# TheShinning/gps-sdr-sim

Hardware: AMD Instinct MI355X
Metric: IQ MSamples/s (and × real-time) at 2.6 MS/s, 12 sats, -b 16; 1/2/4/8 GPU (higher is better)
Workload: dtype int64 phases + f16 x f16 -> f32 MFMA accumulate (exact integer sums)

## Files before the change

### gps-sdr-sim_amd/csrc/common/gss_lin.h

```cpp
#ifndef GSS_LIN_H
#define GSS_LIN_H

#include <stdint.h>

#ifndef GSS_LIN_CH
#define GSS_LIN_CH     16
#endif
#define GSS_LIN_CHUNK  (64 * GSS_LIN_CH)
#define GSS_LIN_SEG    4096

#if defined(__HIPCC__)
#define GSS_LIN_FN static __host__ __device__ inline
#else
#define GSS_LIN_FN static inline
#endif

#define GSS_LIN_CSH    26

GSS_LIN_FN uint32_t gss_lin_dx(uint64_t xs) { return (uint32_t)((xs * 64u + (1ull << 31)) >> 32); }
GSS_LIN_FN uint32_t gss_lin_dz(uint64_t zs)
{
    return (uint32_t)((zs * 64u + (1ull << (GSS_LIN_CSH - 1))) >> GSS_LIN_CSH);
}
GSS_LIN_FN uint64_t gss_lin_xa(uint64_t xs)
// ... 4 lines not shown
GSS_LIN_FN uint64_t gss_lin_za(uint64_t zs)
{
    const int64_t ec = (int64_t)(((uint64_t)gss_lin_dz(zs) << GSS_LIN_CSH) - zs * 64u);
    return (1ull << (GSS_LIN_CSH - 1)) - (uint64_t)((ec * (GSS_LIN_CH - 1)) / 2);
}

GSS_LIN_FN uint32_t gss_lin_e0(uint64_t chips)
{
    const uint32_t e = (uint32_t)(chips % 1023u);
    return e ? e : 1023u;
}

#define GSS_LIN_KDEV_CARR(zs)                                                                      \
    ((((uint64_t)GSS_LIN_CH / 2 + 3) << 31) +                                                     \
     ((2 + (((uint64_t)gss_lin_dz(zs) * (GSS_LIN_CH - 1)) >> 32)) << 32))
#define GSS_LIN_KDEV_CODE (((uint64_t)GSS_LIN_CH / 2 + 3) << (GSS_LIN_CSH - 1))
#define GSS_LIN_WIN_OK(zs) ((zs) * 63u + (3ull << 50) <= (31ull << 50))

#define GSS_LIN_TWE     2560
#define GSS_LIN_CBW_PRE 2
GSS_LIN_FN uint32_t gss_lin_wstep16(int n_per_blk)
{
    return (uint32_t)((104755200ull + (uint64_t)n_per_blk / 2) / (uint64_t)n_per_blk);
}
GSS_LIN_FN int gss_lin_win16_ok(uint64_t zs, int n_per_blk)
{
    const int64_t U = (int64_t)1 << 50, z = (int64_t)zs;
    const int64_t kd = (int64_t)GSS_LIN_KDEV_CODE + ((int64_t)1 << 27);
    const uint32_t w = gss_lin_wstep16(n_per_blk);
    if (zs == 0 || zs >= (uint64_t)U)
        return 0;
    for (int s = 0; s < GSS_LIN_CH; s++) {
        const int64_t f = (int64_t)(((uint64_t)s * w) >> 4) - GSS_LIN_CBW_PRE;
        if (64 * s * z - kd < f * U)
            return 0;
        if (U + (64 * s + 63) * z + kd > (f + 32) * U)
            return 0;
    }
    return 1025 * U + (int64_t)(GSS_LIN_SEG - GSS_LIN_CHUNK) * z + kd < (int64_t)GSS_LIN_TWE * U;
}

GSS_LIN_FN uint64_t gss_lin_lane(uint64_t xs, uint64_t zs, uint32_t l)
{
    const uint32_t lx = (uint32_t)(((uint64_t)l * xs + (1ull << 31)) >> 32);
    const uint32_t lz = (uint32_t)(((uint64_t)l * zs) >> GSS_LIN_CSH);
    return ((uint64_t)lx << 32) | lz;
// ... 147 lines not shown
```

### gps-sdr-sim_amd/csrc/hip/gss_dev.h

```cpp
#ifndef GSS_DEV_H
#define GSS_DEV_H

#include <hip/hip_runtime.h>
#include <stdint.h>
#include "gpssim_amd.h"
#include "../common/gss_impair.h"

extern "C" int gss_fail(int code, const char *fmt, ...);

#define HIP_TRY(x)                                                                           \
    do {                                                                                     \
        hipError_t e_ = (x);                                                                 \
        if (e_ != hipSuccess)                                                                \
            return gss_fail(GSS_E_HIP, "HIP error %s at %s:%d", hipGetErrorString(e_),      \
                            __FILE__, __LINE__);                                             \
    } while (0)

template <class T> struct gss_buf {
    T *p = nullptr;
    size_t cap = 0;
    int reserve(size_t bytes, const char *what)
    {
        if (bytes <= cap)
            return 0;
        release();
        if (hipMalloc((void **)&p, bytes) != hipSuccess) {
            p = nullptr;
            return gss_fail(GSS_E_NOMEM, "%s: %zu bytes of device memory", what, bytes);
        }
// ... 15 lines not shown
    uint32_t ca[32 * GSS_CA_WORDS];
    int16_t lut[1024];
    int32_t noise[GSS_IMP_TBL];
};

struct gss_trk_state;

struct gss_dev {
    int ordinal;
    int seg_r = 1024;
    struct anchor_set {
        gss_buf<double> carr, code;
        gss_buf<uint32_t> cnt;
    } set[2];
    static constexpr int RING = 256;
    hipEvent_t ev_a[RING][2], ev_b[RING][2];
    hipEvent_t ev_l[RING][2];
    int n_a = 0, n_b = 0, n_l = 0;
    lut_arg lut;
    gss_buf<gss_dev_tables> tab;
    gss_buf<uint8_t> d_in, d_out;
    gss_buf<double> d_cend;
    gss_buf<uint32_t> d_cbw;
    gss_buf<int32_t> d_status;
    hipStream_t aux = nullptr;
    hipEvent_t ev_in = nullptr, ev_fb = nullptr;
    struct {
        gss_buf<int8_t> planes, rep;
        gss_buf<uint64_t> rows, cand;
        gss_buf<int32_t> maxes;
    } acq;
    struct {
        gss_buf<gss_trk_state> state;
        gss_buf<gss_trk_job_t> jobs;
    } trk;
};

#endif
```

### gps-sdr-sim_amd/csrc/hip/gss_run.hip

```cpp
#include <hip/hip_runtime.h>
#include <math.h>
#include <stdint.h>
#include <stdlib.h>
#include <stdio.h>
#include <string.h>
#include <time.h>
#include <condition_variable>
#include <mutex>
#include <thread>
#include <unordered_map>
#include <vector>
#include "gpssim_amd.h"
#include "gss_run_modes.h"

extern "C" int gss_fail(int code, const char *fmt, ...);
extern "C" void gss_pool_select(int id);
extern "C" int gss_jam_check(const gss_jam_t *jam, int n_jam);
int run_copy_launch(void *dst, const void *src, size_t n, hipStream_t st);
extern "C" __attribute__((weak)) int gss_impair_device(gss_dev *d, const gss_impair_t *p,
                                                       const int16_t *iq, uint64_t sample0,
                                                       size_t n, int fmt, void *out,
                                                       void *stream);
extern "C" __attribute__((weak)) int gss_jam_device(gss_dev *d, const gss_impair_t *p,
                                                    const gss_jam_t *jam, int n_jam,
                                                    const int16_t *iq, uint64_t sample0, size_t n,
                                                    int fmt, void *out, void *stream);

#define RUN_TRY(x)                                                                           \
    do {                                                                                     \
        hipError_t e_ = (x);                                                                 \
        if (e_ != hipSuccess)                                                                \
            return gss_fail(GSS_E_HIP, "HIP error %s at %s:%d", hipGetErrorString(e_),      \
                            __FILE__, __LINE__);                                             \
    } while (0)

namespace {

static double tnow()
{
    timespec ts;
    clock_gettime(CLOCK_MONOTONIC, &ts);
    return ts.tv_sec + 1e-9 * ts.tv_nsec;
}
static int trace_on()
{
    static int on = -1;
    if (on < 0) {
        const char *e = getenv("GSS_RUN_TRACE");
        on = e && e[0] == '1';
// ... 239 lines not shown
    hipEvent_t tq = nullptr;
    hipEvent_t tk = nullptr;
    hipEvent_t tc = nullptr;
    hipStream_t pst = nullptr;
    hipEvent_t navd = nullptr;
    hipEvent_t proved = nullptr;
    int gpu_proven = 0;
};

struct Run {
    explicit Run(const RunModes &modes) : m(modes) {}
    const RunModes m;
    gss_scn *scn;
    gss_dev *dev = nullptr;
    int ordinal = 0;
    int batch, threads, n_per_blk, carrier_int;
    int fmt = 0;
    size_t bb = 0, bb_r = 0;
    hipStream_t st = nullptr;
    hipStream_t cp[NCOPY] = {};
    uint32_t *d_ca = nullptr;
    hipStream_t nav_st = nullptr;
    hipEvent_t t_base = nullptr;
    hipEvent_t ca_ready = nullptr;
    int64_t first, last;
    int64_t start = 0;
    const gss_run_opts_t *opts;
    const gss_impair_t *impair = nullptr;
    gss_jam_t jam[GSS_MAXJAM];
    int n_jam = 0;
    int fmt_out = 0;
    std::vector<gss_chan_blk_t> pre_blk;
    std::vector<int32_t> pre_nch;
    std::vector<double> pre_ck;
    int64_t pre_n = 0, pre_at = 0;
    std::mutex mu;
    std::condition_variable cv;
    int abort = 0;
    uint32_t ca[32 * GSS_CA_WORDS];
    int nav_planned = 0;
    uint32_t *d_nav = nullptr;
    size_t d_nav_cap = 0;
    struct SpecBatch {
        std::vector<gss_chan_blk_t> blk;
        std::vector<int32_t> nch;
        std::vector<gss_chain_t> chain;
// ... 1133 lines not shown
    }
}


#define THEN(e, x)                                                                           \
    do {                                                                                     \
        if ((e) == hipSuccess)                                                               \
            (e) = (x);                                                                       \
    } while (0)

int run_alloc(Run &r)
{
    gss_ca_table(r.ca);
    hipError_t e = dev_alloc((void **)&r.d_ca, sizeof r.ca);
    THEN(e, r.m.render_rest ? cu_mask_stream(&r.st, r.m.spec_cus, true) : stream_get(&r.st, false));
    for (hipStream_t &c : r.cp)
        THEN(e, stream_get(&c, false));
    if (trace_on()) {
        THEN(e, hipEventCreate(&r.t_base));
        THEN(e, hipEventRecord(r.t_base, r.st));
    }
    if (e != hipSuccess)
        return gss_fail(GSS_E_HIP, "run setup failed");
    return gss_ca_table_device(r.dev, r.d_ca, r.st);
}

void run_release_tables(Run &r)
{
    dev_free(r.d_ca);
    dev_free(r.d_nav);
}

void run_release_streams(Run &r)
{
    stream_put(r.st);
    for (hipStream_t c : r.cp)
        stream_put(c);
    if (r.t_base) (void)hipEventDestroy(r.t_base);
}

int slot_alloc(const Run &r, Slot &sl)
{
    const size_t nb = (size_t)r.batch;
    const unsigned ev = trace_on() ? hipEventDefault : hipEventDisableTiming;
    hipError_t e = pin_alloc((void **)&sl.blk, sizeof(gss_chan_blk_t) * GSS_MAXCH * nb);
    THEN(e, pin_alloc((void **)&sl.nch, sizeof(int32_t) * nb));
    THEN(e, pin_alloc((void **)&sl.ck, sizeof(double) * GSS_MAXCH * GSS_NCK * nb));
    THEN(e, pool_get((void **)&sl.h_out, r.bb * nb, true, r.ordinal, &sl.h_out_bytes));
    THEN(e, pin_alloc((void **)&sl.h_status, sizeof(int32_t)));
    THEN(e, pool_get((void **)&sl.d_out, r.bb_r * nb, false, r.ordinal, &sl.d_out_bytes));
    if (r.impair && r.fmt != r.fmt_out)
// ... 304 lines not shown
```

### gps-sdr-sim_amd/csrc/hip/gss_synth.hip

```cpp
#include <hip/hip_runtime.h>
#include <stdint.h>
#include <stdlib.h>
#include <string.h>
#include "gpssim_amd.h"
#include "gss_dev.h"
#include "../common/gss_phase.h"
#include "../common/gss_lin.h"

#define SYNTH_THREADS  256
#define SYNTH_WAVES    (SYNTH_THREADS / 64)
#define ANCHOR_THREADS 64
#define CHUNK_BYTES    128
#define CHUNK_PIECES   (CHUNK_BYTES / 16)
#define LUT_N          1024

__global__ __launch_bounds__(ANCHOR_THREADS) void gss_anchor_kernel(
    const gss_chan_blk_t *__restrict__ blk, const int32_t *__restrict__ nch,
    const double *__restrict__ carr_ck, int nblk, int nchp, int n_per_blk, int nseg, int nsegp,
    int seg_r, double *__restrict__ seg_carr, double *__restrict__ seg_code,
    uint32_t *__restrict__ seg_cnt, double *__restrict__ carr_end,
    const int32_t *__restrict__ blist)
{
    const int nsub = carr_ck ? GSS_NCK : 1;
    const int nbw = (nblk + ANCHOR_THREADS - 1) / ANCHOR_THREADS;
// ... 346 lines not shown
                                    (size_t)ch * CHUNK_BYTES + piece * 16;
                    const uint32_t *sp = stg + src * (CHUNK_BYTES / 4) + piece * 4;
                    store16(sdst, make_uint4(sp[0], sp[1], sp[2], sp[3]));
                }
            }
            wave_sync_lds();
        }
        if (!full && nsamp > 0) {
            int nbytes = nsamp * BPS4 / 4;
            uint8_t *bp = dst + (size_t)ch * CHUNK_BYTES;
            const uint8_t *sp = (const uint8_t *)mine;
            for (int i = 0; i < nbytes; i++)
                bp[i] = sp[i];
        }
    }
    if (bad && status)
        atomicOr(status, bad);
}

#define LIN_THREADS 256
#define LIN_WAVES   (LIN_THREADS / 64)
#define LIN_STEPS   (GSS_LIN_SEG / 64)
#define LIN_CH      GSS_LIN_CH
#define CBW_PRE     2
#define CBW_CHIPS   3072
#define CAB_W       ((CBW_CHIPS + 96) / 32)
static_assert(LIN_STEPS % LIN_CH == 0 && (LIN_CH & (LIN_CH - 1)) == 0, "whole chunks");
#define LIN_SW_SGPRS 68
typedef _Float16 lin_half4 __attribute__((ext_vector_type(4)));
typedef _Float16 lin_half8 __attribute__((ext_vector_type(8)));
typedef float lin_f4 __attribute__((ext_vector_type(4)));
#define LIN_GS    2
#define LIN_MAGF  (12582912.0f + 64.0f * LIN_GS)
#define LIN_MAGB  0x4B400000u

#define LIN_CHUNKS (LIN_STEPS / LIN_CH)
struct alignas(16) lin_ck {
    uint64_t B[GSS_MAXCH];
    uint32_t A[GSS_MAXCH / 2][5][4];
};
struct alignas(16) lin_wrec {
    uint64_t D[GSS_MAXCH];
    int32_t gd[GSS_MAXCH];
    int32_t pos1[GSS_MAXCH];
    lin_ck ck[LIN_CHUNKS];
};
static_assert(LIN_CHUNKS * GSS_MAXCH == 64, "one lane per (chunk, channel) record");
static_assert(offsetof(lin_wrec, D) % 16 == 0 && offsetof(lin_wrec, ck) % 16 == 0 &&
              offsetof(lin_ck, B) % 16 == 0 && offsetof(lin_ck, A) % 16 == 0 &&
              sizeof(lin_ck) % 16 == 0, "16-byte reads of a pair's B, D and gain operand");

typedef gss_lin_row lin_seg;
typedef gss_lin_chan lin_chan;
static_assert(sizeof(lin_seg) == 32 && sizeof(lin_chan) == 32, "two 16-byte LDS reads each");

__global__ void gss_cab_kernel(const uint32_t *__restrict__ ca_bits, int n_ca,
                               uint32_t *__restrict__ cab)
{
    const int i = blockIdx.x * blockDim.x + threadIdx.x;
    if (i >= n_ca * CAB_W)
        return;
    const int row = i / CAB_W, j0 = (i - row * CAB_W) * 32 - 32;
    const uint32_t *cb = ca_bits + (size_t)row * GSS_CA_WORDS;
    uint32_t w = 0;
    for (int q = 0; q < 32; q++) {
        const int e = j0 + q, chip = ((e % GSS_CA_LEN) + GSS_CA_LEN) % GSS_CA_LEN;
        w |= (((cb[chip >> 5] >> (chip & 31)) & 1u) ^ 1u) << q;
    }
    cab[i] = w;
}

__global__ void gss_tw16_kernel(const uint32_t *__restrict__ cab, int n_ca, uint32_t w,
                                uint32_t *__restrict__ tw)
{
    const int i = blockIdx.x * blockDim.x + threadIdx.x;
    if (i >= n_ca * GSS_LIN_TWE * LIN_CH)
        return;
    const int row = i / (GSS_LIN_TWE * LIN_CH), r = i - row * (GSS_LIN_TWE * LIN_CH);
    const int E = r / LIN_CH, st = r % LIN_CH;
    const uint32_t j = min((uint32_t)(E + (int)(((uint32_t)st * w) >> 4) - GSS_LIN_CBW_PRE + 32),
                           (uint32_t)(32 * CAB_W - 64));
    const uint32_t *c = cab + (size_t)row * CAB_W;
    const uint32_t lin = __builtin_amdgcn_alignbit(c[(j >> 5) + 1], c[j >> 5], j & 31);
    tw[i] = __builtin_amdgcn_alignbit(lin, lin, (32u - j) & 31u);
}

struct lin_wsrc {
    const uint32_t *W;
};

__device__ __forceinline__ void lin_wissue(const lin_wsrc &w, uint32_t (&ws)[LIN_CH])
{
#pragma unroll
    for (int s = 0; s < LIN_CH; s++)
        ws[s] = w.W[s];
}

__device__ __forceinline__ void lin_wfence(const uint32_t (&ws)[LIN_CH])
{
    static_assert(LIN_CH == 16, "the fence below names 16 windows");
    asm volatile("" :: "s"(ws[0]), "s"(ws[1]), "s"(ws[2]), "s"(ws[3]), "s"(ws[4]), "s"(ws[5]),
                 "s"(ws[6]), "s"(ws[7]), "s"(ws[8]), "s"(ws[9]), "s"(ws[10]), "s"(ws[11]),
                 "s"(ws[12]), "s"(ws[13]), "s"(ws[14]), "s"(ws[15]));
}

__device__ __forceinline__ lin_wsrc lin_wsrc_of(uint32_t wa, const uint32_t *__restrict__ tw)
{
// ... 574 lines not shown
    }
    *out = d;
    return 0;
}

extern "C" int gss_dev_close(gss_dev *d)
{
    if (!d) return 0;
    (void)hipSetDevice(d->ordinal);
    gss_run_pool_drain(d->ordinal);
    for (auto &a : d->set) {
        a.carr.release();
        a.code.release();
        a.cnt.release();
    }
    if (d->aux) (void)hipStreamDestroy(d->aux);
    if (d->ev_in) (void)hipEventDestroy(d->ev_in);
    if (d->ev_fb) (void)hipEventDestroy(d->ev_fb);
    d->tab.release();
    d->d_in.release();
    d->d_out.release();
    d->d_cend.release();
    d->d_cbw.release();
    d->d_status.release();
    d->acq.planes.release();
    d->acq.rep.release();
    d->acq.rows.release();
    d->acq.cand.release();
    d->acq.maxes.release();
    d->trk.state.release();
    d->trk.jobs.release();
    for (int i = 0; i < gss_dev::RING; i++)
        for (int j = 0; j < 2; j++) {
            if (d->ev_a[i][j]) (void)hipEventDestroy(d->ev_a[i][j]);
            if (d->ev_b[i][j]) (void)hipEventDestroy(d->ev_b[i][j]);
            if (d->ev_l[i][j]) (void)hipEventDestroy(d->ev_l[i][j]);
        }
    delete d;
    return 0;
}

static int nseg_of(int n, int r) { return (n + r - 1) / r; }
static int nsegp_of(int n, int r) { return (nseg_of(n, r) + 1 + 31) & ~31; }

static int reserve_set(gss_dev *d, int set, int max_blocks, int n_per_blk, int R)
{
// ... 123 lines not shown
                                 const int32_t *nch, int nch_max, const uint32_t *ca_bits,
                                 int n_ca, const uint32_t *nav, int n_nav, int nblk,
                                 int n_per_blk, int fmt, void *out, int32_t *status, void *stream)
{
    (void)n_ca; (void)n_nav;
    return render_launch(d, set, blk, nch, nch_max, ca_bits, nav, nblk, n_per_blk, fmt, out,
                         status, nullptr, d->seg_r, stream);
}

typedef void (*lin_fn)(const gss_lin_t *, const gss_chan_blk_t *, const int32_t *,
                       const int32_t *, const uint32_t *, const uint32_t *, const uint4 *, int,
                       int, uint8_t *, size_t);

static lin_fn pick_lin(int fmt)
{
    switch (fmt) {
    case 16: return gss_lin_kernel<16>;
    case 8: return gss_lin_kernel<8>;
    case 1: return gss_lin_kernel<1>;
    default: return nullptr;
    }
}

extern "C" int gss_synth_lin_device(gss_dev *d, const gss_chan_blk_t *blk, const int32_t *nch,
                                    int nch_max, const gss_lin_t *lin, const int32_t *fast,
                                    const int32_t *fb_list, int n_fb, const double *carr_ck,
                                    const uint32_t *ca_bits, int n_ca, const uint32_t *nav,
                                    int n_nav, int nblk, int n_per_blk, int fmt, void *out,
                                    int32_t *status, void *stream)
{
    (void)n_nav;
    if (!d || !blk || !nch || !lin || !fast || !ca_bits || !out || nblk <= 0 || n_per_blk <= 0 ||
        n_ca <= 0 || n_fb < 0 || n_fb > nblk || (n_fb > 0 && !fb_list))
        return gss_fail(GSS_E_ARG, "invalid synth_lin arguments");
    const size_t bb = gss_block_bytes(n_per_blk, fmt);
    if (bb == 0)
        return gss_fail(GSS_E_ARG, "invalid format %d for %d samples/block", fmt, n_per_blk);
    const int nchp = nch_max < 1 ? 1 : nch_max;
    if (nchp > GSS_MAXCH)
        return gss_fail(GSS_E_ARG, "nch_max %d > %d", nch_max, GSS_MAXCH);
    lin_fn fn = pick_lin(fmt);
    if (!fn)
        return gss_fail(GSS_E_ARG, "no fast kernel for fmt=%d nch=%d", fmt, nchp);
    HIP_TRY(hipSetDevice(d->ordinal));
    hipStream_t st = (hipStream_t)stream;
    const size_t ncbw = (size_t)n_ca * CAB_W, ntw = (size_t)n_ca * GSS_LIN_TWE * LIN_CH;
    const size_t tw_off = (ncbw + 63) & ~(size_t)63;
    int rc = d->d_cbw.reserve((tw_off + ntw) * sizeof(uint32_t), "chip-sign streams");
    if (rc) return rc;
    hipLaunchKernelGGL(gss_cab_kernel, dim3((unsigned)((ncbw + 255) / 256)), dim3(256), 0, st,
                       ca_bits, n_ca, d->d_cbw.p);
    HIP_TRY(hipGetLastError());
    hipLaunchKernelGGL(gss_tw16_kernel, dim3((unsigned)((ntw + 255) / 256)), dim3(256), 0, st,
                       (const uint32_t *)d->d_cbw.p, n_ca, gss_lin_wstep16(n_per_blk),
                       d->d_cbw.p + tw_off);
    HIP_TRY(hipGetLastError());
    const int segs = (n_per_blk + 64 * LIN_STEPS - 1) / (64 * LIN_STEPS);
    const int wg_per_blk = (segs + LIN_WAVES - 1) / LIN_WAVES;
    if (n_fb > 0) {
        HIP_TRY(hipEventRecord(d->ev_in, st));
        HIP_TRY(hipStreamWaitEvent(d->aux, d->ev_in, 0));
        const int R = 256;
        rc = anchor_launch(d, 0, blk, nch, nch_max, carr_ck, n_fb, n_per_blk, nullptr,
                               fb_list, R, d->aux);
        if (rc) return rc;
        rc = render_launch(d, 0, blk, nch, nch_max, ca_bits, nav, n_fb, n_per_blk, fmt, out,
                           status, fb_list, R, d->aux);
        if (rc) return rc;
        HIP_TRY(hipEventRecord(d->ev_fb, d->aux));
    }
    hipEvent_t *ev = d->ev_l[d->n_l % gss_dev::RING];
    d->n_l++;
    HIP_TRY(hipEventRecord(ev[0], st));
    hipLaunchKernelGGL(fn, dim3((unsigned)nblk * wg_per_blk), dim3(LIN_THREADS), 0, st, lin,
                       blk, nch, fast, d->d_cbw.p, d->d_cbw.p + tw_off, (const uint4 *)d->tab.p->lut16,
                       n_per_blk, wg_per_blk, (uint8_t *)out, bb);
    HIP_TRY(hipGetLastError());
    HIP_TRY(hipEventRecord(ev[1], st));
    if (n_fb > 0)
        HIP_TRY(hipStreamWaitEvent(st, d->ev_fb, 0));
    return 0;
}

extern "C" int gss_synth_device(gss_dev *d, const gss_chan_blk_t *blk, const int32_t *nch,
                                int nch_max, const double *carr_ck, const uint32_t *ca_bits,
                                int n_ca,
                                const uint32_t *nav, int n_nav, int nblk, int n_per_blk, int fmt,
                                void *out, double *carr_end, int32_t *status, void *stream)
{
    if (!d || !blk || !nch || !ca_bits || !out || nblk <= 0 || n_per_blk <= 0)
        return gss_fail(GSS_E_ARG, "invalid synth arguments");
    if (gss_block_bytes(n_per_blk, fmt) == 0)
        return gss_fail(GSS_E_ARG, "invalid format %d for %d samples/block", fmt, n_per_blk);
    int rc = gss_anchor_device(d, 0, blk, nch, nch_max, carr_ck, nblk, n_per_blk, carr_end,
                               stream);
    if (rc) return rc;
    return gss_render_device(d, 0, blk, nch, nch_max, ca_bits, n_ca, nav, n_nav, nblk, n_per_blk,
                             fmt, out, status, stream);
// ... 166 lines not shown
```

### gps-sdr-sim_amd/gpssim_amd/__init__.py

```python
import ctypes as C
import os

import numpy as np

PKG_DIR = os.path.dirname(os.path.dirname(os.path.abspath(__file__)))
REPO_DIR = os.path.dirname(PKG_DIR)
_INTREE = os.path.join(PKG_DIR, "lib", "libgpssim_amd.so")
if os.environ.get("GSS_LIB_PATH") and os.environ.get("GSS_ALLOW_LIB_OVERRIDE") != "1":
    raise ImportError("GSS_LIB_PATH is set without GSS_ALLOW_LIB_OVERRIDE=1: refusing to load a "
                      "library other than the in-tree build " + _INTREE)
LIB_PATH = os.environ.get("GSS_LIB_PATH") or _INTREE
IN_TREE = os.path.abspath(LIB_PATH) == os.path.abspath(_INTREE)
CLI_PATH = os.path.join(PKG_DIR, "bin", "gps-sdr-sim")
ACQ_CLI_PATH = os.path.join(PKG_DIR, "bin", "gps-sdr-acq")
TRK_CLI_PATH = os.path.join(PKG_DIR, "bin", "gps-sdr-track")
PVT_CLI_PATH = os.path.join(PKG_DIR, "bin", "gps-sdr-pvt")

MAXCH = 16
CA_WORDS = 32
NAV_WORDS = 60
NCK = 8
FMT_SC01, FMT_SC08, FMT_SC16 = 1, 8, 16

CHAN_DTYPE = np.dtype([
# ... 196 lines not shown
SINK_FN = C.CFUNCTYPE(C.c_int, C.c_void_p, C.c_void_p, C.c_size_t, C.c_int64, C.c_int)
_SIGS = {
    "gss_run": (C.c_int, [_P, _P, C.c_int64, C.c_int64, C.c_int, C.c_int, SINK_FN, _P]),
    "gss_run_ex": (C.c_int, [_P, _P, C.c_int64, C.c_int64, C.c_int, C.c_int, SINK_FN, _P, _P]),
    "gss_dev_open": (C.c_int, [C.POINTER(_P), C.c_int]),
    "gss_dev_close": (C.c_int, [_P]),
    "gss_dev_reserve": (C.c_int, [_P, C.c_int, C.c_int]),
    "gss_block_bytes": (C.c_size_t, [C.c_int, C.c_int]),
    "gss_anchor_device": (C.c_int, [_P, C.c_int, _P, _P, C.c_int, _P, C.c_int, C.c_int, _P,
                                    _P]),
    "gss_render_device": (C.c_int, [_P, C.c_int, _P, _P, C.c_int, _P, C.c_int, _P, C.c_int,
                                    C.c_int, C.c_int, C.c_int, _P, _P, _P]),
    "gss_synth_device": (C.c_int, [_P, _P, _P, C.c_int, _P, _P, C.c_int, _P, C.c_int,
                                   C.c_int, C.c_int, C.c_int, _P, _P, _P, _P]),
    "gss_synth_host": (C.c_int, [_P, _P, _P, _P, _P, C.c_int, _P, C.c_int, C.c_int, C.c_int,
                                 C.c_int, _P, _P]),
    "gss_linearize": (C.c_int, [_P, _P, C.c_int, C.c_int, _P, C.c_int, _P, C.c_int, _P, _P,
                                C.c_int]),
    "gss_linearize_device": (C.c_int, [_P, _P, _P, C.c_int, C.c_int, _P, C.c_int, _P, C.c_int, _P,
                                       _P, _P]),
    "gss_synth_lin_device": (C.c_int, [_P, _P, _P, C.c_int, _P, _P, _P, C.c_int, _P, _P,
                                       C.c_int, _P, C.c_int, C.c_int, C.c_int, C.c_int, _P, _P,
                                       _P]),
    "gss_minmax_mod": (None, [C.c_uint64, C.c_uint64, C.c_uint64, C.c_uint64,
                              C.POINTER(C.c_uint64), C.POINTER(C.c_uint64)]),
    "gss_first_below": (C.c_uint64, [C.c_uint64] * 5),
    "gss_hits_mod": (C.c_int, [C.c_uint64] * 5 + [_P, C.c_int, C.c_int]),
    "gss_noise_table": (C.c_int, [_P]),
    "gss_impair_host": (C.c_int, [C.POINTER(Impair), _P, C.c_uint64, C.c_size_t, C.c_int, _P]),
    "gss_impair_device": (C.c_int, [_P, C.POINTER(Impair), _P, C.c_uint64, C.c_size_t, C.c_int,
                                    _P, _P]),
    "gss_jam_make": (C.c_int, [C.c_double] * 7 + [C.POINTER(Jam)]),
    "gss_jam_host": (C.c_int, [C.POINTER(Impair), C.POINTER(Jam), C.c_int, _P, C.c_uint64,
                               C.c_size_t, C.c_int, _P]),
    "gss_jam_device": (C.c_int, [_P, C.POINTER(Impair), C.POINTER(Jam), C.c_int, _P, C.c_uint64,
                                 C.c_size_t, C.c_int, _P, _P]),
    "gss_acq_sizes": (C.c_int, [C.POINTER(Acq), C.POINTER(C.c_int32), C.POINTER(C.c_int32),
                                C.POINTER(C.c_int64), C.POINTER(C.c_int32),
                                C.POINTER(C.c_int32)]),
    "gss_acquire_host": (C.c_int, [C.POINTER(Acq), _P, _P, _P, C.POINTER(C.c_int), C.c_int]),
    "gss_acquire_device": (C.c_int, [_P, C.POINTER(Acq), _P, _P, _P, _P, _P]),
    "gss_acquire": (C.c_int, [_P, C.POINTER(Acq), _P, _P, _P, C.POINTER(C.c_int)]),
    "gss_acq_expect": (C.c_int, [_P, C.c_double, C.c_int64, C.POINTER(_Truth)]),
    "gss_acq_threshold": (C.c_double, [C.c_int, C.c_uint64, C.c_double]),
    "gss_trk_defaults": (C.c_int, [C.c_int32, C.c_int32, C.POINTER(Trk)]),
    "gss_trk_job_from_peak": (C.c_int, [C.POINTER(Acq), _P, C.c_int64, C.c_int32, _P]),
# ... 686 lines not shown
        return (out, cend) if want_carr_end else out

    def synth_device(self, blk_ptr, nch_ptr, nch_max, ca_ptr, n_ca, nav_ptr, n_nav, nblk,
                     n_per_blk, fmt, out_ptr, carr_end_ptr=0, status_ptr=0, stream=0, ck_ptr=0):
        _check(lib().gss_synth_device(self._h, blk_ptr, nch_ptr, nch_max, ck_ptr or None, ca_ptr,
                                      n_ca, nav_ptr,
                                      n_nav, nblk, n_per_blk, fmt, out_ptr,
                                      carr_end_ptr or None, status_ptr or None, stream or None))

    def ca_table_device(self, out_ptr, stream=0):
        _check(lib().gss_ca_table_device(self._h, out_ptr, stream or None))

    def nav_rows_device(self, src_ptr, first, n, rows_ptr, stream=0):
        _check(lib().gss_nav_rows_device(self._h, src_ptr, first, n, rows_ptr, stream or None))

    def synth_lin_device(self, blk_ptr, nch_ptr, nch_max, lin_ptr, fast_ptr, fb_ptr, n_fb, ca_ptr,
                         n_ca, nav_ptr, n_nav, nblk, n_per_blk, fmt, out_ptr, status_ptr=0,
                         stream=0, ck_ptr=0):
        _check(lib().gss_synth_lin_device(self._h, blk_ptr, nch_ptr, nch_max, lin_ptr, fast_ptr,
                                          fb_ptr or None, n_fb, ck_ptr or None, ca_ptr, n_ca,
                                          nav_ptr, n_nav, nblk, n_per_blk, fmt, out_ptr,
                                          status_ptr or None, stream or None))

    def timing_lin(self):
        n, t = C.c_int(), C.c_float()
        _check(lib().gss_dev_timing_lin(self._h, C.byref(n), C.byref(t)))
        return n.value, t.value

    def anchor_device(self, set_, blk_ptr, nch_ptr, nch_max, nblk, n_per_blk, ck_ptr=0,
                      carr_end_ptr=0, stream=0):
        _check(lib().gss_anchor_device(self._h, set_, blk_ptr, nch_ptr, nch_max, ck_ptr or None,
                                       nblk, n_per_blk, carr_end_ptr or None, stream or None))

    def render_device(self, set_, blk_ptr, nch_ptr, nch_max, ca_ptr, n_ca, nav_ptr, n_nav, nblk,
                      n_per_blk, fmt, out_ptr, status_ptr=0, stream=0):
        _check(lib().gss_render_device(self._h, set_, blk_ptr, nch_ptr, nch_max, ca_ptr, n_ca,
                                       nav_ptr, n_nav, nblk, n_per_blk, fmt, out_ptr,
                                       status_ptr or None, stream or None))

    def impair_device(self, imp, iq_ptr, sample0, n, fmt, out_ptr, stream=0):
        _check(lib().gss_impair_device(self._h, C.byref(imp), C.c_void_p(iq_ptr), int(sample0),
                                       int(n), int(fmt), C.c_void_p(out_ptr),
                                       C.c_void_p(stream or None)))

    def jam_device(self, imp, jam, iq_ptr, sample0, n, fmt, out_ptr, stream=0):
        arr, nj = _jam_array(jam)
# ... 116 lines not shown
```

### gps-sdr-sim_amd/gpssim_amd/render.py

```python
import time

import numpy as np

from . import (CHAN_DTYPE, LIN_DTYPE, MAXCH, NCK, block_bytes, ca_table, carr_advance_ck,
               linearize)


def block_checkpoints(blk, nch, n_per_blk, blocks=None):
    ck = np.zeros((len(nch), MAXCH, NCK), np.float64)
    for b in (range(len(nch)) if blocks is None else blocks):
        for k in range(int(nch[b])):
            ck[b, k] = carr_advance_ck(float(blk[b, k]["carr0"]), float(blk[b, k]["carr_step"]),
                                       n_per_blk)[1]
    return ck


class DeviceWindow:

    def __init__(self, torch, dev, dev_t, blk, nch, nav, n_per_blk, fmt, ck=None, threads=8,
                 batch=3000, out=None, proof="gpu", sizes=None):
        self.torch, self.dev, self.fmt, self.npb = torch, dev, fmt, n_per_blk

        def up(a):
            return torch.from_numpy(np.ascontiguousarray(a).view(np.uint8).reshape(-1)).to(dev_t)

        t0 = time.perf_counter()
        if proof == "gpu":
            self.d_blk, self.d_nch = up(blk), up(np.asarray(nch, np.int32))
            ca = ca_table()
            self.d_ca, self.d_nav = up(ca), up(nav)
            nb = len(nch)
            self.d_lin = torch.empty(max(1, nb * MAXCH * LIN_DTYPE.itemsize), dtype=torch.uint8,
                                     device=dev_t)
            d_fast = torch.empty(max(1, nb), dtype=torch.int32, device=dev_t)
            stream = torch.cuda.current_stream(dev_t).cuda_stream
            if nb:
                dev.linearize_device(self.d_blk.data_ptr(), self.d_nch.data_ptr(), nb, n_per_blk,
                                     self.d_ca.data_ptr(), len(ca), self.d_nav.data_ptr(),
                                     len(nav), self.d_lin.data_ptr(), d_fast.data_ptr(), stream)
            fast = d_fast[:nb].cpu().numpy()
            lin = None
        else:
            lin, fast = linearize(blk, nch, nav, n_per_blk, threads=threads)
        self.lin_s = time.perf_counter() - t0
        self.proof = proof
        self.nblk = len(nch)
        self.n_fast = int(fast.sum())
        self.ch_samples_fast = int(np.asarray(nch)[fast.astype(bool)].astype(np.int64).sum()) * \
            int(n_per_blk)
        self.nch_max = int(nch.max()) if len(nch) else 1
        ca = ca_table()
        self.n_ca, self.n_nav = len(ca), len(nav)
        self.bb = block_bytes(n_per_blk, fmt)

        if ck is None and self.n_fast < self.nblk:
            ck = block_checkpoints(blk, nch, n_per_blk, np.nonzero(fast == 0)[0])
        if lin is not None:
            self.d_blk, self.d_nch, self.d_lin = up(blk), up(nch), up(lin)
            self.d_ca, self.d_nav = up(ca), up(nav)
        self.d_ck = up(ck) if ck is not None else None
        self.d_fast = up(np.asarray(fast, np.int32))
        self.out = out if out is not None else torch.empty(self.nblk * self.bb, dtype=torch.uint8,
                                                           device=dev_t)
        assert self.out.numel() >= self.nblk * self.bb
        self.batches = []
        if sizes is None:
            sizes = [min(batch, self.nblk - b0) for b0 in range(0, self.nblk, batch)]
        assert sum(sizes) == self.nblk and all(n > 0 for n in sizes)
        b1 = 0
        for n in sizes:
            b0, b1 = b1, b1 + n
            fb = np.nonzero(fast[b0:b1] == 0)[0].astype(np.int32)
            d_fb = torch.from_numpy(fb if len(fb) else np.zeros(1, np.int32)).to(dev_t)
            self.batches.append((b0, b1, d_fb, len(fb)))
        if self.nblk:
            dev.reserve(max(sizes), n_per_blk)

    def step(self, stream=0, lin=None, fast=None):
        for i in range(len(self.batches)):
            self.step_batch(i, stream, lin, fast)

    def step_batch(self, i, stream=0, lin=None, fast=None):
        cs, ls, ks = CHAN_DTYPE.itemsize * MAXCH, LIN_DTYPE.itemsize * MAXCH, 8 * MAXCH * NCK
        d_lin = self.d_lin if lin is None else lin
        d_fast = self.d_fast if fast is None else fast
        for b0, b1, d_fb, n_fb in self.batches[i:i + 1]:
            self.dev.synth_lin_device(
                self.d_blk.data_ptr() + b0 * cs, self.d_nch.data_ptr() + b0 * 4, self.nch_max,
                d_lin.data_ptr() + b0 * ls, d_fast.data_ptr() + b0 * 4,
                d_fb.data_ptr(), n_fb, self.d_ca.data_ptr(), self.n_ca, self.d_nav.data_ptr(),
                self.n_nav, b1 - b0, self.npb, self.fmt, self.out.data_ptr() + b0 * self.bb,
                stream=stream,
                ck_ptr=(self.d_ck.data_ptr() + b0 * ks) if self.d_ck is not None else 0)

    def free_inputs(self):
        for a in ("d_blk", "d_nch", "d_lin", "d_ck", "d_ca", "d_nav", "d_fast"):
            setattr(self, a, None)
        self.batches = []

    def free(self, release=True):
        self.free_inputs()
        self.out = None
        if release:
            self.torch.cuda.empty_cache()
```

### include/gpssim_amd.h

```cpp
#ifndef GPSSIM_AMD_H
#define GPSSIM_AMD_H

#include <stdint.h>
#include <stddef.h>

#ifdef __cplusplus
extern "C" {
#endif

#define GSS_MAXCH      16
#define GSS_CA_LEN     1023
#define GSS_CA_WORDS   32
#define GSS_NAV_WORDS  60

#define GSS_FMT_SC01   1
#define GSS_FMT_SC08   8
#define GSS_FMT_SC16   16

#define GSS_OK           0
#define GSS_E_ARG       -1
#define GSS_E_HIP       -2
#define GSS_E_NOMEM     -3
#define GSS_E_IO        -4
#define GSS_E_INPUT     -5
// ... 42 lines not shown
#define GSS_NPATCH 8
typedef struct gss_lin {
    uint64_t x0, xs;
    uint64_t z0, zs;
    int64_t pdelta[GSS_NPATCH];
    int32_t gpos[GSS_NGC];
    int32_t gval[GSS_NGC];
    int32_t ppos[GSS_NPATCH];
} gss_lin_t;

int gss_linearize(const gss_chan_blk_t *blk, const int32_t *nch, int nblk, int n_per_blk,
                  const uint32_t *ca_bits, int n_ca, const uint32_t *nav, int n_nav,
                  gss_lin_t *lin, int32_t *fast, int threads);

int gss_linearize_device(gss_dev *d, const gss_chan_blk_t *blk, const int32_t *nch, int nblk,
                         int n_per_blk, const uint32_t *ca_bits, int n_ca, const uint32_t *nav,
                         int n_nav, gss_lin_t *lin, int32_t *fast, void *stream);

int gss_synth_lin_device(gss_dev *d, const gss_chan_blk_t *blk, const int32_t *nch, int nch_max,
                         const gss_lin_t *lin, const int32_t *fast, const int32_t *fb_list,
                         int n_fb, const double *carr_ck, const uint32_t *ca_bits, int n_ca,
                         const uint32_t *nav, int n_nav, int nblk, int n_per_blk, int fmt,
                         void *out, int32_t *status, void *stream);

void gss_minmax_mod(uint64_t n, uint64_t m, uint64_t a, uint64_t s, uint64_t *mn, uint64_t *mx);
uint64_t gss_first_below(uint64_t n, uint64_t m, uint64_t a, uint64_t s, uint64_t w);
int gss_hits_mod(uint64_t n, uint64_t lgB, uint64_t a0, uint64_t st, uint64_t w, int64_t *hit,
                 int cap, int scan);

int gss_synth_host(gss_dev *d, const gss_chan_blk_t *blk, const int32_t *nch,
                   const double *carr_ck, const uint32_t *ca_bits, int n_ca, const uint32_t *nav, int n_nav,
                   int nblk, int n_per_blk, int fmt, void *out, double *carr_end);

typedef struct gss_impair {
    uint64_t seed;
    uint32_t sigma_q8;
    int32_t  shift;
} gss_impair_t;

int gss_noise_table(int32_t *out);
int gss_impair_host(const gss_impair_t *p, const int16_t *iq, uint64_t sample0, size_t n,
                    int fmt, void *out);
int gss_impair_device(gss_dev *d, const gss_impair_t *p, const int16_t *iq, uint64_t sample0,
                      size_t n, int fmt, void *out, void *stream);

#define GSS_MAXJAM 4
// ... 371 lines not shown
```

Baseline: 554,900.

## Cache per-device chip-window tables across synth calls and build them directly from CA bits

Precomputes the 16-step chip-window tables once per (CA table pointer, code count, step width) key, stores them in a small LRU set on the device, and reuses them in every synth_lin call. Before this, each batch rebuilt them with two kernels. The separate intermediate chip-sign stream kernel is removed: table entries are now computed straight from the CA bit rows by a shared helper. This takes per-batch table-build launches off the hot loop, at the cost of extra device memory, pointer-keyed cache invalidation, and device synchronizations when tables are dropped or replaced.

```diff
diff --git a/gps-sdr-sim_amd/csrc/common/gss_lin.h b/gps-sdr-sim_amd/csrc/common/gss_lin.h
--- a/gps-sdr-sim_amd/csrc/common/gss_lin.h
+++ b/gps-sdr-sim_amd/csrc/common/gss_lin.h
@@ -50,6 +50,26 @@
 GSS_LIN_FN uint32_t gss_lin_wstep16(int n_per_blk)
 {
     return (uint32_t)((104755200ull + (uint64_t)n_per_blk / 2) / (uint64_t)n_per_blk);
+}
+GSS_LIN_FN uint32_t gss_lin_ca32(const uint32_t *row_bits, uint32_t c)
+{
+    const uint32_t i = c >> 5, sh = c & 31u;
+    const uint32_t lo = row_bits[i], hi = i < 31u ? row_bits[i + 1] : 0u;
+    uint32_t v = sh ? (lo >> sh) | (hi << (32u - sh)) : lo;
+    if (c > 1023u - 32u) {
+        const uint32_t k = 1023u - c;
+        v = (v & ((1u << k) - 1u)) | (row_bits[0] << k);
+    }
+    return v;
+}
+#define GSS_LIN_TWE_MAX 3072
+GSS_LIN_FN uint32_t gss_lin_tw16_entry(const uint32_t *row_bits, uint32_t E, uint32_t s, uint32_t w)
+{
+    uint32_t j = E + ((s * w) >> 4) - GSS_LIN_CBW_PRE + 32u;
+    j = j < GSS_LIN_TWE_MAX + 32u ? j : GSS_LIN_TWE_MAX + 32u;
+    const uint32_t v = ~gss_lin_ca32(row_bits, (j + (1023u - 32u)) % 1023u);
+    const uint32_t r = j & 31u;
+    return r ? (v << r) | (v >> (32u - r)) : v;
 }
 GSS_LIN_FN int gss_lin_win16_ok(uint64_t zs, int n_per_blk)
 {
diff --git a/gps-sdr-sim_amd/csrc/hip/gss_dev.h b/gps-sdr-sim_amd/csrc/hip/gss_dev.h
--- a/gps-sdr-sim_amd/csrc/hip/gss_dev.h
+++ b/gps-sdr-sim_amd/csrc/hip/gss_dev.h
@@ -5,6 +5,7 @@
 #include <stdint.h>
 #include "gpssim_amd.h"
 #include "../common/gss_impair.h"
+#include "gss_lin_sets.h"
 
 extern "C" int gss_fail(int code, const char *fmt, ...);
 
@@ -66,6 +67,12 @@
     gss_buf<uint8_t> d_in, d_out;
     gss_buf<double> d_cend;
     gss_buf<uint32_t> d_cbw;
+    struct lin_table {
+        gss_buf<uint32_t> tw;
+        hipEvent_t built = nullptr;
+        bool ready = false;
+    } lin_tab[GSS_LIN_NSETS];
+    gss_lin_sets lin_sets;
     gss_buf<int32_t> d_status;
     hipStream_t aux = nullptr;
     hipEvent_t ev_in = nullptr, ev_fb = nullptr;
diff --git a/gps-sdr-sim_amd/csrc/hip/gss_lin_sets.h b/gps-sdr-sim_amd/csrc/hip/gss_lin_sets.h
--- /dev/null
+++ b/gps-sdr-sim_amd/csrc/hip/gss_lin_sets.h
@@ -0,0 +1,61 @@
+#ifndef GSS_LIN_SETS_H
+#define GSS_LIN_SETS_H
+
+#include <stdint.h>
+
+#define GSS_LIN_NSETS 4
+
+struct gss_lin_key {
+    const void *ca;
+    int n_ca;
+    uint32_t w;
+};
+
+struct gss_lin_sets {
+    struct slot {
+        gss_lin_key key;
+        uint64_t seq;
+        bool used;
+    } s[GSS_LIN_NSETS] = {};
+    uint64_t seq = 0;
+
+    int find(const gss_lin_key &k) const
+    {
+        for (int i = 0; i < GSS_LIN_NSETS; i++)
+            if (s[i].used && s[i].key.ca == k.ca && s[i].key.n_ca == k.n_ca && s[i].key.w == k.w)
+                return i;
+        return -1;
+    }
+    int place(bool *replaces) const
+    {
+        int old = 0;
+        for (int i = 0; i < GSS_LIN_NSETS; i++) {
+            if (!s[i].used) {
+                *replaces = false;
+                return i;
+            }
+            if (s[i].seq < s[old].seq)
+                old = i;
+        }
+        *replaces = true;
+        return old;
+    }
+    void take(int i, const gss_lin_key &k)
+    {
+        s[i].key = k;
+        s[i].seq = ++seq;
+        s[i].used = true;
+    }
+    int forget(const void *ca)
+    {
+        int n = 0;
+        for (int i = 0; i < GSS_LIN_NSETS; i++)
+            if (s[i].used && (!ca || s[i].key.ca == ca)) {
+                s[i].used = false;
+                n++;
+            }
+        return n;
+    }
+};
+
+#endif
diff --git a/gps-sdr-sim_amd/csrc/hip/gss_run.hip b/gps-sdr-sim_amd/csrc/hip/gss_run.hip
--- a/gps-sdr-sim_amd/csrc/hip/gss_run.hip
+++ b/gps-sdr-sim_amd/csrc/hip/gss_run.hip
@@ -25,6 +25,9 @@
                                                     const gss_jam_t *jam, int n_jam,
                                                     const int16_t *iq, uint64_t sample0, size_t n,
                                                     int fmt, void *out, void *stream);
+extern "C" __attribute__((weak)) int gss_lin_tables_device(gss_dev *d, const uint32_t *ca_bits,
+                                                           int n_ca, int n_per_blk, void *stream);
+extern "C" __attribute__((weak)) int gss_lin_tables_drop(gss_dev *d, const uint32_t *ca_bits);
 
 #define RUN_TRY(x)                                                                           \
     do {                                                                                     \
@@ -310,6 +313,7 @@
     uint32_t *d_ca = nullptr;
     hipStream_t nav_st = nullptr;
     hipEvent_t t_base = nullptr;
+    bool ca_prepared = false;
     hipEvent_t ca_ready = nullptr;
     int64_t first, last;
     int64_t start = 0;
@@ -1489,11 +1493,19 @@
     }
     if (e != hipSuccess)
         return gss_fail(GSS_E_HIP, "run setup failed");
-    return gss_ca_table_device(r.dev, r.d_ca, r.st);
+    int rc = gss_ca_table_device(r.dev, r.d_ca, r.st);
+    if (!rc && r.m.use_lin && gss_lin_tables_device && gss_lin_tables_drop) {
+        rc = gss_lin_tables_device(r.dev, r.d_ca, 32, r.n_per_blk, r.st);
+        r.ca_prepared = rc == 0;
+    }
+    return rc;
 }
 
 void run_release_tables(Run &r)
 {
+    if (r.ca_prepared)
+        (void)gss_lin_tables_drop(r.dev, r.d_ca);
+    r.ca_prepared = false;
     dev_free(r.d_ca);
     dev_free(r.d_nav);
 }
diff --git a/gps-sdr-sim_amd/csrc/hip/gss_synth.hip b/gps-sdr-sim_amd/csrc/hip/gss_synth.hip
--- a/gps-sdr-sim_amd/csrc/hip/gss_synth.hip
+++ b/gps-sdr-sim_amd/csrc/hip/gss_synth.hip
@@ -392,9 +392,6 @@
 #define LIN_WAVES   (LIN_THREADS / 64)
 #define LIN_STEPS   (GSS_LIN_SEG / 64)
 #define LIN_CH      GSS_LIN_CH
-#define CBW_PRE     2
-#define CBW_CHIPS   3072
-#define CAB_W       ((CBW_CHIPS + 96) / 32)
 static_assert(LIN_STEPS % LIN_CH == 0 && (LIN_CH & (LIN_CH - 1)) == 0, "whole chunks");
 #define LIN_SW_SGPRS 68
 typedef _Float16 lin_half4 __attribute__((ext_vector_type(4)));
@@ -424,35 +421,15 @@
 typedef gss_lin_chan lin_chan;
 static_assert(sizeof(lin_seg) == 32 && sizeof(lin_chan) == 32, "two 16-byte LDS reads each");
 
-__global__ void gss_cab_kernel(const uint32_t *__restrict__ ca_bits, int n_ca,
-                               uint32_t *__restrict__ cab)
-{
-    const int i = blockIdx.x * blockDim.x + threadIdx.x;
-    if (i >= n_ca * CAB_W)
-        return;
-    const int row = i / CAB_W, j0 = (i - row * CAB_W) * 32 - 32;
-    const uint32_t *cb = ca_bits + (size_t)row * GSS_CA_WORDS;
-    uint32_t w = 0;
-    for (int q = 0; q < 32; q++) {
-        const int e = j0 + q, chip = ((e % GSS_CA_LEN) + GSS_CA_LEN) % GSS_CA_LEN;
-        w |= (((cb[chip >> 5] >> (chip & 31)) & 1u) ^ 1u) << q;
-    }
-    cab[i] = w;
-}
-
-__global__ void gss_tw16_kernel(const uint32_t *__restrict__ cab, int n_ca, uint32_t w,
+__global__ void gss_tw16_kernel(const uint32_t *__restrict__ ca_bits, int n_ca, uint32_t w,
                                 uint32_t *__restrict__ tw)
 {
     const int i = blockIdx.x * blockDim.x + threadIdx.x;
     if (i >= n_ca * GSS_LIN_TWE * LIN_CH)
         return;
     const int row = i / (GSS_LIN_TWE * LIN_CH), r = i - row * (GSS_LIN_TWE * LIN_CH);
-    const int E = r / LIN_CH, st = r % LIN_CH;
-    const uint32_t j = min((uint32_t)(E + (int)(((uint32_t)st * w) >> 4) - GSS_LIN_CBW_PRE + 32),
-                           (uint32_t)(32 * CAB_W - 64));
-    const uint32_t *c = cab + (size_t)row * CAB_W;
-    const uint32_t lin = __builtin_amdgcn_alignbit(c[(j >> 5) + 1], c[j >> 5], j & 31);
-    tw[i] = __builtin_amdgcn_alignbit(lin, lin, (32u - j) & 31u);
+    tw[i] = gss_lin_tw16_entry(ca_bits + (size_t)row * GSS_CA_WORDS, (uint32_t)(r / LIN_CH),
+                               (uint32_t)(r % LIN_CH), w);
 }
 
 struct lin_wsrc {
@@ -1073,6 +1050,11 @@
     d->d_out.release();
     d->d_cend.release();
     d->d_cbw.release();
+    (void)gss_lin_tables_drop(d, nullptr);
+    for (auto &t : d->lin_tab) {
+        t.tw.release();
+        if (t.built) (void)hipEventDestroy(t.built);
+    }
     d->d_status.release();
     d->acq.planes.release();
     d->acq.rep.release();
@@ -1242,6 +1224,55 @@
     }
 }
 
+static int lin_table_build(const uint32_t *ca_bits, int n_ca, int n_per_blk,
+                           gss_buf<uint32_t> &buf, hipStream_t st)
+{
+    const size_t ntw = (size_t)n_ca * GSS_LIN_TWE * LIN_CH;
+    int rc = buf.reserve(ntw * sizeof(uint32_t), "chunk window table");
+    if (rc) return rc;
+    hipLaunchKernelGGL(gss_tw16_kernel, dim3((unsigned)((ntw + 255) / 256)), dim3(256), 0, st,
+                       ca_bits, n_ca, gss_lin_wstep16(n_per_blk), buf.p);
+    HIP_TRY(hipGetLastError());
+    return 0;
+}
+
+extern "C" int gss_lin_tables_device(gss_dev *d, const uint32_t *ca_bits, int n_ca, int n_per_blk,
+                                     void *stream)
+{
+    if (!d || !ca_bits || n_ca <= 0 || n_per_blk <= 0)
+        return gss_fail(GSS_E_ARG, "invalid lin_tables arguments");
+    const gss_lin_key key{ca_bits, n_ca, gss_lin_wstep16(n_per_blk)};
+    if (d->lin_sets.find(key) >= 0)
+        return 0;
+    HIP_TRY(hipSetDevice(d->ordinal));
+    bool replaces = false;
+    const int i = d->lin_sets.place(&replaces);
+    gss_dev::lin_table &t = d->lin_tab[i];
+    if (replaces) {
+        HIP_TRY(hipDeviceSynchronize());
+        d->lin_sets.s[i].used = false;
+    }
+    if (!t.built)
+        HIP_TRY(hipEventCreateWithFlags(&t.built, hipEventDisableTiming));
+    int rc = lin_table_build(ca_bits, n_ca, n_per_blk, t.tw, (hipStream_t)stream);
+    if (rc) return rc;
+    HIP_TRY(hipEventRecord(t.built, (hipStream_t)stream));
+    t.ready = false;
+    d->lin_sets.take(i, key);
+    return 0;
+}
+
+extern "C" int gss_lin_tables_drop(gss_dev *d, const uint32_t *ca_bits)
+{
+    if (!d)
+        return gss_fail(GSS_E_ARG, "null device");
+    if (d->lin_sets.forget(ca_bits) > 0) {
+        HIP_TRY(hipSetDevice(d->ordinal));
+        HIP_TRY(hipDeviceSynchronize());
+    }
+    return 0;
+}
+
 extern "C" int gss_synth_lin_device(gss_dev *d, const gss_chan_blk_t *blk, const int32_t *nch,
                                     int nch_max, const gss_lin_t *lin, const int32_t *fast,
                                     const int32_t *fb_list, int n_fb, const double *carr_ck,
@@ -1264,17 +1295,23 @@
         return gss_fail(GSS_E_ARG, "no fast kernel for fmt=%d nch=%d", fmt, nchp);
     HIP_TRY(hipSetDevice(d->ordinal));
     hipStream_t st = (hipStream_t)stream;
-    const size_t ncbw = (size_t)n_ca * CAB_W, ntw = (size_t)n_ca * GSS_LIN_TWE * LIN_CH;
-    const size_t tw_off = (ncbw + 63) & ~(size_t)63;
-    int rc = d->d_cbw.reserve((tw_off + ntw) * sizeof(uint32_t), "chip-sign streams");
-    if (rc) return rc;
-    hipLaunchKernelGGL(gss_cab_kernel, dim3((unsigned)((ncbw + 255) / 256)), dim3(256), 0, st,
-                       ca_bits, n_ca, d->d_cbw.p);
-    HIP_TRY(hipGetLastError());
-    hipLaunchKernelGGL(gss_tw16_kernel, dim3((unsigned)((ntw + 255) / 256)), dim3(256), 0, st,
-                       (const uint32_t *)d->d_cbw.p, n_ca, gss_lin_wstep16(n_per_blk),
-                       d->d_cbw.p + tw_off);
-    HIP_TRY(hipGetLastError());
+    const uint32_t *tw = nullptr;
+    const int ts = d->lin_sets.find(gss_lin_key{ca_bits, n_ca, gss_lin_wstep16(n_per_blk)});
+    if (ts >= 0) {
+        gss_dev::lin_table &t = d->lin_tab[ts];
+        if (!t.ready) {
+            t.ready = hipEventQuery(t.built) == hipSuccess;
+            (void)hipGetLastError();
+        }
+        if (!t.ready)
+            HIP_TRY(hipStreamWaitEvent(st, t.built, 0));
+        tw = t.tw.p;
+    } else {
+        int rc = lin_table_build(ca_bits, n_ca, n_per_blk, d->d_cbw, st);
+        if (rc) return rc;
+        tw = d->d_cbw.p;
+    }
+    int rc = 0;
     const int segs = (n_per_blk + 64 * LIN_STEPS - 1) / (64 * LIN_STEPS);
     const int wg_per_blk = (segs + LIN_WAVES - 1) / LIN_WAVES;
     if (n_fb > 0) {
@@ -1293,7 +1330,7 @@
     d->n_l++;
     HIP_TRY(hipEventRecord(ev[0], st));
     hipLaunchKernelGGL(fn, dim3((unsigned)nblk * wg_per_blk), dim3(LIN_THREADS), 0, st, lin,
-                       blk, nch, fast, d->d_cbw.p, d->d_cbw.p + tw_off, (const uint4 *)d->tab.p->lut16,
+                       blk, nch, fast, (const uint32_t *)nullptr, tw, (const uint4 *)d->tab.p->lut16,
                        n_per_blk, wg_per_blk, (uint8_t *)out, bb);
     HIP_TRY(hipGetLastError());
     HIP_TRY(hipEventRecord(ev[1], st));
diff --git a/gps-sdr-sim_amd/gpssim_amd/__init__.py b/gps-sdr-sim_amd/gpssim_amd/__init__.py
--- a/gps-sdr-sim_amd/gpssim_amd/__init__.py
+++ b/gps-sdr-sim_amd/gpssim_amd/__init__.py
@@ -242,6 +242,8 @@
     "gss_synth_lin_device": (C.c_int, [_P, _P, _P, C.c_int, _P, _P, _P, C.c_int, _P, _P,
                                        C.c_int, _P, C.c_int, C.c_int, C.c_int, C.c_int, _P, _P,
                                        _P]),
+    "gss_lin_tables_device": (C.c_int, [_P, _P, C.c_int, C.c_int, _P]),
+    "gss_lin_tables_drop": (C.c_int, [_P, _P]),
     "gss_minmax_mod": (None, [C.c_uint64, C.c_uint64, C.c_uint64, C.c_uint64,
                               C.POINTER(C.c_uint64), C.POINTER(C.c_uint64)]),
     "gss_first_below": (C.c_uint64, [C.c_uint64] * 5),
@@ -974,6 +976,12 @@
                                           nav_ptr, n_nav, nblk, n_per_blk, fmt, out_ptr,
                                           status_ptr or None, stream or None))
 
+    def lin_tables_device(self, ca_ptr, n_ca, n_per_blk, stream=0):
+        _check(lib().gss_lin_tables_device(self._h, ca_ptr, n_ca, n_per_blk, stream or None))
+
+    def lin_tables_drop(self, ca_ptr=0):
+        _check(lib().gss_lin_tables_drop(self._h, ca_ptr or None))
+
     def timing_lin(self):
         n, t = C.c_int(), C.c_float()
         _check(lib().gss_dev_timing_lin(self._h, C.byref(n), C.byref(t)))
diff --git a/gps-sdr-sim_amd/gpssim_amd/render.py b/gps-sdr-sim_amd/gpssim_amd/render.py
--- a/gps-sdr-sim_amd/gpssim_amd/render.py
+++ b/gps-sdr-sim_amd/gpssim_amd/render.py
@@ -17,9 +17,12 @@
 
 class DeviceWindow:
 
+    _ca_ptr = 0
+
     def __init__(self, torch, dev, dev_t, blk, nch, nav, n_per_blk, fmt, ck=None, threads=8,
-                 batch=3000, out=None, proof="gpu", sizes=None):
+                 batch=3000, out=None, proof="gpu", sizes=None, ca=None):
         self.torch, self.dev, self.fmt, self.npb = torch, dev, fmt, n_per_blk
+        ca = np.ascontiguousarray(ca_table() if ca is None else ca, np.uint32)
 
         def up(a):
             return torch.from_numpy(np.ascontiguousarray(a).view(np.uint8).reshape(-1)).to(dev_t)
@@ -27,7 +30,6 @@
         t0 = time.perf_counter()
         if proof == "gpu":
             self.d_blk, self.d_nch = up(blk), up(np.asarray(nch, np.int32))
-            ca = ca_table()
             self.d_ca, self.d_nav = up(ca), up(nav)
             nb = len(nch)
             self.d_lin = torch.empty(max(1, nb * MAXCH * LIN_DTYPE.itemsize), dtype=torch.uint8,
@@ -41,7 +43,7 @@
             fast = d_fast[:nb].cpu().numpy()
             lin = None
         else:
-            lin, fast = linearize(blk, nch, nav, n_per_blk, threads=threads)
+            lin, fast = linearize(blk, nch, nav, n_per_blk, threads=threads, ca=ca)
         self.lin_s = time.perf_counter() - t0
         self.proof = proof
         self.nblk = len(nch)
@@ -49,7 +51,6 @@
         self.ch_samples_fast = int(np.asarray(nch)[fast.astype(bool)].astype(np.int64).sum()) * \
             int(n_per_blk)
         self.nch_max = int(nch.max()) if len(nch) else 1
-        ca = ca_table()
         self.n_ca, self.n_nav = len(ca), len(nav)
         self.bb = block_bytes(n_per_blk, fmt)
 
@@ -75,6 +76,10 @@
             self.batches.append((b0, b1, d_fb, len(fb)))
         if self.nblk:
             dev.reserve(max(sizes), n_per_blk)
+        self._ca_ptr = self.d_ca.data_ptr()
+        dev.lin_tables_drop(self._ca_ptr)
+        dev.lin_tables_device(self._ca_ptr, self.n_ca, n_per_blk,
+                              torch.cuda.current_stream(dev_t).cuda_stream)
 
     def step(self, stream=0, lin=None, fast=None):
         for i in range(len(self.batches)):
@@ -93,7 +98,13 @@
                 stream=stream,
                 ck_ptr=(self.d_ck.data_ptr() + b0 * ks) if self.d_ck is not None else 0)
 
+    def _drop_tables(self):
+        ptr, self._ca_ptr = self._ca_ptr, 0
+        if ptr and self.dev._h:
+            self.dev.lin_tables_drop(ptr)
+
     def free_inputs(self):
+        self._drop_tables()
         for a in ("d_blk", "d_nch", "d_lin", "d_ck", "d_ca", "d_nav", "d_fast"):
             setattr(self, a, None)
         self.batches = []
@@ -103,3 +114,9 @@
         self.out = None
         if release:
             self.torch.cuda.empty_cache()
+
+    def __del__(self):
+        try:
+            self._drop_tables()
+        except Exception:
+            pass
diff --git a/include/gpssim_amd.h b/include/gpssim_amd.h
--- a/include/gpssim_amd.h
+++ b/include/gpssim_amd.h
@@ -88,6 +88,10 @@
                          int n_fb, const double *carr_ck, const uint32_t *ca_bits, int n_ca,
                          const uint32_t *nav, int n_nav, int nblk, int n_per_blk, int fmt,
                          void *out, int32_t *status, void *stream);
+
+int gss_lin_tables_device(gss_dev *d, const uint32_t *ca_bits, int n_ca, int n_per_blk,
+                          void *stream);
+int gss_lin_tables_drop(gss_dev *d, const uint32_t *ca_bits);
 
 void gss_minmax_mod(uint64_t n, uint64_t m, uint64_t a, uint64_t s, uint64_t *mn, uint64_t *mx);
 uint64_t gss_first_below(uint64_t n, uint64_t m, uint64_t a, uint64_t s, uint64_t w);
```

Measured after the change: 556,100, median of 6. No clear change (+0.2%).
